# team-ergo-unipi/ergo_uvo

Hardware: AMD Instinct MI355X
Metric: stereo frame-pairs/sec (detect+match+pose) @1920x1080, 3k kpts (higher is better)
Workload: dtype f32+f64

## Files before the change

### ergo_uvo_amd/csrc/surf.hip

```cpp
#include "uvo_ctx.h"
#include <type_traits>
#include <string.h>
#include "uvo_math.h"
#include <algorithm>
#include <utility>
#include <vector>
#include <string>

namespace uvo {

struct ImgPair { const uint8_t* img[2]; int32_t* sum[2]; int32_t* planes[2]; int pw, pstride; int* cand_n; int* big_n; int* surv_n; };
struct AreaTab;
struct CandOut { uvo_keypoint* cand[2]; int* count; int cap; };
struct SurvOut { Survivor* list; int* count; int cap; };
static_assert(sizeof(Survivor) == 128, "a survivor record is 32 words");
struct SortArgs { const uvo_keypoint* cand[2]; const int* cand_n; uvo_keypoint* out[2]; int* out_n[2]; int* rank; int cap;
                  int4* big_par; int* big_n; int* gate_nqa; int gate_min_features; };
struct DescArgs { const uint8_t* img[2]; uvo_keypoint* kps[2]; float* desc[2]; const int* n[2]; const float* DW;
                  const int4* big_par; const int* big_n; const int* big_large; int cap;
                  const AreaTab* tabs; const int* iscale;
                  int extended;
                  const int32_t* sum[2]; const float* ori_w; int* ori_drop; };
struct LaneArgs { ImgPair ip; int32_t* part; SurvOut sv; CandOut out; SortArgs sa; DescArgs da; uint8_t* patch; const int4* big_in; int4* big_out; int* big_large; };
struct LanePair { LaneArgs a[2]; };
// ... 454 lines not shown

template <int O, int L>
__device__ __forceinline__ float plane_pp(ImgRsrc rs, int voff, int pw, int pstride)
{
    using LC = LayerC<OctC<O>::size(L)>;
#define SVP(dy, dx) (int)__builtin_amdgcn_raw_buffer_load_b32(rs, voff + 4 * ((dx) >> 2) + plane_written<(dy), (dx)>(), 4 * ((((dy) & 3) * 4 + ((dx) & 3)) * pstride + ((dy) >> 2) * pw), 0)
    UVO_HESSIAN_CONSTS(LC);
    float pp;
    UVO_HESSIAN_PP(SVP, pp)
    return pp;
}
template <int O, int L>
__device__ __forceinline__ float plane_det(ImgRsrc rs, int voff, int pw, int pstride, float pp)
{
    using LC = LayerC<OctC<O>::size(L)>;
    UVO_HESSIAN_CONSTS(LC);
    float det;
    UVO_HESSIAN_DXY(SVP, pp, det)
#undef SVP
    return det;
}
template <int O, int TW, int TH, int NT, class OP>
__device__ __forceinline__ void det_layers_p3(const int32_t* __restrict__ planes, int pw, int pstride, float* __restrict__ sdet,
                                              const OP& op, int px0, int py0, float skip_thr)
{
    using OC = OctC<O>;
    constexpr int Q = OC::STEP / 4;
    const ImgRsrc rs = img_rsrc(reinterpret_cast<const uint8_t*>(planes), 16 * pstride * 4);
    const int tid = lane_tid();
#pragma unroll
    for (int it = 0; it < (TW * TH + NT - 1) / NT; it++) {
        const int sidx = tid + it * NT;
        if ((it + 1) * NT > TW * TH && sidx >= TW * TH) break;
        const int ry = sidx / TW, rx = sidx - ry * TW;
        bool ok[3]; int voff[3]; float pp[3], det[3];
#pragma unroll
        for (int l = 0; l < 3; l++) {
            const int m = l == 0 ? OC::margin(1) : l == 1 ? OC::margin(2) : OC::margin(3);
            const auto& lp = op.L[l + 1];
            const int oi = py0 + ry - m, oj = px0 + rx - m;
            ok[l] = oi >= 0 && oi < lp.samples_i && oj >= 0 && oj < lp.samples_j;
            voff[l] = ok[l] ? 4 * ((oi * Q) * pw + oj * Q) : 0x7FFFFFF0;
        }
        pp[0] = plane_pp<O, 1>(rs, voff[0], pw, pstride);
        pp[1] = plane_pp<O, 2>(rs, voff[1], pw, pstride);
        pp[2] = plane_pp<O, 3>(rs, voff[2], pw, pstride);
        const bool n0 = ok[0] && pp[0] > skip_thr, n1 = ok[1] && pp[1] > skip_thr, n2 = ok[2] && pp[2] > skip_thr;
        det[0] = ok[0] ? kDetBelow : 0.f; det[1] = ok[1] ? kDetBelow : 0.f; det[2] = ok[2] ? kDetBelow : 0.f;
        if (n0 || n1 || n2) {
            const float d0 = plane_det<O, 1>(rs, n0 ? voff[0] : 0x7FFFFFF0, pw, pstride, pp[0]);
            const float d1 = plane_det<O, 2>(rs, n1 ? voff[1] : 0x7FFFFFF0, pw, pstride, pp[1]);
            const float d2 = plane_det<O, 3>(rs, n2 ? voff[2] : 0x7FFFFFF0, pw, pstride, pp[2]);
            if (n0) det[0] = d0;
            if (n1) det[1] = d1;
            if (n2) det[2] = d2;
        }
#pragma unroll
        for (int l = 0; l < 3; l++) sdet[(l * TH + ry) * TW + rx] = det[l];
    }
}


template <int TW, int TH>
struct NmsLds { static constexpr int kList = 3 * ((TW - 1) / 2) * ((TH - 1) / 2), kWords = kList + 2; };

#ifndef UVO_STAMPS
#define UVO_STAMPS 0
#endif
__device__ long long* g_hess_stamps = nullptr;
__device__ __forceinline__ void hess_stamp(int k, long long v = -1)
{
#if UVO_STAMPS
    long long* st = g_hess_stamps;
    if (st && threadIdx.x == 0) st[((size_t)blockIdx.y * gridDim.x + blockIdx.x) * 8 + k] = v >= 0 ? v : (long long)wall_clock64();
#endif
}
template <int TW, int TH>
__device__ __forceinline__ void nms_zero(unsigned* s_list) { if (lane_tid() == 0) reinterpret_cast<int*>(s_list + NmsLds<TW, TH>::kList)[0] = 0; }
template <int TW, int TH, int NT, class OP>
__device__ __forceinline__ void nms_survivors(const float* __restrict__ sdet, unsigned* __restrict__ s_list, const OP& op, float thr,
                                              int px0, int py0, int im, const SurvOut& sv)
{
    const int tid = lane_tid();
    int* s_n = reinterpret_cast<int*>(s_list + NmsLds<TW, TH>::kList);
    static_assert((TW & (TW - 1)) == 0 && NT % TW == 0 && TW <= 64, "tile width: a power of two that divides the workgroup, a row within a wave");
    constexpr int G = NT / TW, ITER = (TH - 2 + G - 1) / G;
    const int rx = tid & (TW - 1), g = tid / TW;
    const int j = px0 + rx;
    float col[3][ITER + 2];
#pragma unroll
    for (int l = 0; l < 3; l++)
#pragma unroll
        for (int k = 0; k < ITER + 2; k++) col[l][k] = sdet[(l * TH + min(g * ITER + k, TH - 1)) * TW + rx];
    float cmax = col[0][1];
#pragma unroll
    for (int l = 0; l < 3; l++)
#pragma unroll
        for (int k = 0; k < ITER; k++) cmax = fmaxf(cmax, col[l][k + 1]);
    if (__any(cmax > thr)) {
    float m3[3][ITER], m3l[3][ITER], m3r[3][ITER];
#pragma unroll
    for (int l = 0; l < 3; l++)
#pragma unroll
        for (int k = 0; k < ITER; k++) {
            const float v = fmaxf(fmaxf(col[l][k], col[l][k + 1]), col[l][k + 2]);
            m3[l][k] = v;
            m3l[l][k] = __int_as_float(__builtin_amdgcn_update_dpp(__float_as_int(v), __float_as_int(v), 0x138, 0xF, 0xF, false));
            m3r[l][k] = __int_as_float(__builtin_amdgcn_update_dpp(__float_as_int(v), __float_as_int(v), 0x130, 0xF, 0xF, false));
        }
#pragma unroll
    for (int l = 0; l < 3; l++) {
        const int L = l + 1;
        const int m = op.nms_margin[l];
        const bool col_ok = op.L[L].samples_i != 0 && op.L[L + 1].samples_i != 0 && rx >= 1 && rx <= TW - 2 && j >= m && j < op.cols - m;
#pragma unroll
        for (int k = 0; k < ITER; k++) {
            const int ry = g * ITER + k + 1, i = py0 + ry;
            const float val0 = col[l][k + 1];
            float nb = fmaxf(fmaxf(col[l][k], col[l][k + 2]), fmaxf(m3l[l][k], m3r[l][k]));
            if (L <= 2) nb = fmaxf(nb, fmaxf(m3[l + 1][k], fmaxf(m3l[l + 1][k], m3r[l + 1][k])));
            if (L >= 2) nb = fmaxf(nb, fmaxf(m3[l - 1][k], fmaxf(m3l[l - 1][k], m3r[l - 1][k])));
            const bool is_max = col_ok && ry <= TH - 2 && i >= m && i < op.rows - m && val0 > thr && val0 > nb;
            if (is_max) s_list[atomicAdd(&s_n[0], 1)] = (unsigned)L | ((unsigned)ry << 8) | ((unsigned)rx << 16);
        }
    }
    }
    hess_stamp(5);
    __syncthreads();
    hess_stamp(6);
    const int nloc = s_n[0];
    if (nloc == 0) return;
    if (tid == 0) s_n[1] = atomicAdd(sv.count, nloc);
    __syncthreads();
    hess_stamp(7);
    const int base = s_n[1];
    for (int e = tid; e < nloc * 32; e += NT) {
        const int t = e >> 5, wd = e & 31;
        if (base + t >= sv.cap) continue;
        Survivor* r = sv.list + base + t;
        const unsigned ent = s_list[t];
        const int L = ent & 255u, ry = (ent >> 8) & 255u, rx = ent >> 16;
        int val;
        if (wd < 5) val = wd == 0 ? im : wd == 1 ? op.octave : wd == 2 ? L : wd == 3 ? py0 + ry : px0 + rx;
        else {
            const int q = wd - 5, row = q / 9, nb9 = q - row * 9;
            const float* d = sdet + ((L - 2 + row) * TH + ry + nb9 / 3 - 1) * TW + rx + nb9 % 3 - 1;
            const bool have = (row == 0 && L >= 2) || row == 1 || (row == 2 && L <= 2);
            val = have ? __float_as_int(*d) : 0;
        }
        reinterpret_cast<int*>(r)[wd] = val;
    }
}

static const int kFinishPerWg = 16;
__global__ __launch_bounds__(256) void k_hessian_finish(LanePair lp, const OctavePat* __restrict__ ops, int w, int h)
{
    const LaneArgs& LA = lp.a[blockIdx.y]; const SurvOut& sv = LA.sv; const ImgPair& ip = LA.ip; const CandOut& out = LA.out;
    __shared__ uvo_keypoint s_kp[2][kFinishPerWg];
    __shared__ int s_cnt[2], s_base[2];
    const int grp = threadIdx.x >> 4, k = threadIdx.x & 15;
    const int n = min(*sv.count, sv.cap);
    if (blockIdx.x == 0 && threadIdx.x == 0 && *sv.count > sv.cap) atomicAdd(&out.count[0], out.cap + 1);
    if (blockIdx.x * kFinishPerWg >= n) return;
    if (threadIdx.x < 2) s_cnt[threadIdx.x] = 0;
    __syncthreads();
    const int sw = w + 1;
#pragma unroll 1
    for (int rd = 0; rd < kFinishPerWg / 16; rd++) {
        const int t = blockIdx.x * kFinishPerWg + rd * 16 + grp;
        if (t >= n) continue;
        const Survivor* r = sv.list + t;
        const int im = r->im, L = r->L, i = r->i, j = r->j;
        const OctavePat& op = ops[r->octave];
        const int step = op.step;
        const int32_t* __restrict__ gsum = ip.sum[im];
        auto exact_det = [&](const LayerPat& lo, int ii, int jj) {
            const int oi = ii - lo.margin, oj = jj - lo.margin;
            float d = 0.f;
            if (oi >= 0 && oi < lo.samples_i && oj >= 0 && oj < lo.samples_j) {
                const int32_t* o = gsum + (size_t)(oi * step) * sw + oj * step;
                float dx, dy, dxy;
                haar_response(lo, [&](int yy, int xx) { return o[(size_t)yy * sw + xx]; }, &dx, &dy, &dxy);
                d = dx * dy - 0.81f * dxy * dxy;
            }
            return d;
        };
        float v2[2];
#pragma unroll
        for (int q = 0; q < 2; q++) {
            const int e = k + 16 * q;
            v2[q] = r->n9[e < 27 ? e : 0];
        }
#pragma unroll 1
        for (int q = 0; q < 2; q++) {
            const int e = k + 16 * q;
            if (e >= 27) continue;
            const int row = e / 9, nb = e - row * 9;
            const bool outer = (L == 1 && row == 0) || (L == 3 && row == 2);
            if (outer || v2[q] == kDetBelow) v2[q] = exact_det(op.L[L - 1 + row], i + nb / 3 - 1, j + nb % 3 - 1);
        }
        const int g0 = (threadIdx.x & 63) & ~15;
        float N9[3][9];
#pragma unroll
        for (int e = 0; e < 27; e++) N9[e / 9][e % 9] = __shfl(v2[e / 16], g0 + (e & 15));
        if (k != 0) continue;
        const float val0 = N9[1][4];
        if (L != 2) {
            bool is_max = true;
#pragma unroll
            for (int b = 0; b < 9; b++) is_max = is_max && (val0 > (L == 1 ? N9[0][b] : N9[2][b]));
            if (!is_max) continue;
        }
        const LayerPat& lp = op.L[L];
        float dx, dy;
        {
            const int32_t* o = gsum + (size_t)((i - lp.margin) * step) * sw + (j - lp.margin) * step;
            haar_response(lp, [&](int yy, int xx) { return o[(size_t)yy * sw + xx]; }, &dx, &dy, nullptr);
        }
        const int ds = lp.size - op.L[L - 1].size;
        uvo_keypoint kp;
        bool ok;
        switch (step) {
        case 1:  ok = make_keypoint<1>(N9, val0, dx + dy, i, j, lp.size, ds, op.octave, w, h, &kp); break;
        case 2:  ok = make_keypoint<2>(N9, val0, dx + dy, i, j, lp.size, ds, op.octave, w, h, &kp); break;
        case 4:  ok = make_keypoint<4>(N9, val0, dx + dy, i, j, lp.size, ds, op.octave, w, h, &kp); break;
        default: ok = make_keypoint<8>(N9, val0, dx + dy, i, j, lp.size, ds, op.octave, w, h, &kp); break;
        }
        if (ok) s_kp[im][atomicAdd(&s_cnt[im], 1)] = kp;
    }
    __syncthreads();
    if (threadIdx.x < 2 && s_cnt[threadIdx.x] > 0) s_base[threadIdx.x] = atomicAdd(&out.count[threadIdx.x], s_cnt[threadIdx.x]);
    __syncthreads();
    for (int e = threadIdx.x; e < 2 * kFinishPerWg; e += 256) {
        const int im = e / kFinishPerWg, q = e - im * kFinishPerWg;
        if (q < s_cnt[im] && s_base[im] + q < out.cap) out.cand[im][s_base[im] + q] = s_kp[im][q];
    }
}

#define UVO_FILL(quads, nt) (((quads) + (nt) - 1) / (nt) <= 6 ? ((quads) + (nt) - 1) / (nt) : 4)
template <int O, int TW, int TH, int NT, class OP>
__device__ __forceinline__ void hessian_nms_c_tile(const ImgPair& ip, int w, int h, const OP& op, float thr, const SurvOut& sv,
                                                   int bx, int by, int im, unsigned char* smem)
{
    using OC = OctC<O>;
    constexpr int STEP = OC::STEP;
    constexpr int TWs = OctTile<O, TW>::TWs;
    constexpr int THs = (TH - 1) * STEP + (OC::HI - OC::LO) + 1;
    constexpr int PW = OctTile<O, TW>::PW;
    const int tid = lane_tid();
    const int sw = w + 1;
    const int32_t* __restrict__ gsum = ip.sum[im];
    float* sdet = reinterpret_cast<float*>(smem);
    int32_t* stile = reinterpret_cast<int32_t*>(smem + sizeof(float) * 3 * TH * TW);

    const int px0 = bx * (TW - 2) - 1, py0 = by * (TH - 2) - 1;
    const int sx0 = px0 * STEP + OC::LO, sy0 = py0 * STEP + OC::LO;
    constexpr int QPR = OctTile<O, TW>::TWq / 4, kQuads = THs * QPR, kFill = UVO_FILL(kQuads, NT), kQ = NT / QPR, kR = NT % QPR;
    static_assert(STEP == 1 || STEP == 2, "tile fill handles octaves 0 and 1");
    static_assert(OctTile<O, TW>::TWq < kSumPad && STEP - OC::LO < kSumPad, "integral slack too small for the tile overshoot");
    int fidx = tid, fty = tid / QPR, fq = tid - fty * QPR;
#pragma unroll 1
    for (int i0 = 0; i0 < kQuads; i0 += NT * kFill) {
        SumQuad v[kFill];
        int dst[kFill];
#pragma unroll
        for (int u = 0; u < kFill; u++) {
            const bool in = fidx < kQuads;
            const int gy = min(max(sy0 + fty, 0), h), gx = sx0 + 4 * fq;
            v[u] = *reinterpret_cast<const SumQuad*>(gsum + (in ? gy * sw + gx : 0));
            dst[u] = in ? fty * STEP * PW + (4 / STEP) * fq : -1;
            fidx += NT; fq += kR; fty += kQ;
            if (fq >= QPR) { fq -= QPR; fty++; }
        }
#pragma unroll
        for (int u = 0; u < kFill; u++) {
            if (dst[u] < 0) continue;
            if constexpr (STEP == 1) {
                *reinterpret_cast<int4*>(stile + dst[u]) = make_int4(v[u].a, v[u].b, v[u].c, v[u].d);
            } else {
                *reinterpret_cast<int2*>(stile + dst[u]) = make_int2(v[u].a, v[u].c);
                *reinterpret_cast<int2*>(stile + dst[u] + PW) = make_int2(v[u].b, v[u].d);
            }
        }
    }
    nms_zero<TW, TH>(reinterpret_cast<unsigned*>(stile + THs * STEP * PW));
    __syncthreads();
    hess_stamp(1);
    det_layer_c<O, 1, TW, TH, NT>(stile, sdet, op, px0, py0, thr);
    det_layer_c<O, 2, TW, TH, NT>(stile, sdet, op, px0, py0, thr);
    det_layer_c<O, 3, TW, TH, NT>(stile, sdet, op, px0, py0, thr);
    __syncthreads();
    hess_stamp(2);
    nms_survivors<TW, TH, NT>(sdet, reinterpret_cast<unsigned*>(stile + THs * STEP * PW), op, thr, px0, py0, im, sv);
}
template <int O, int TW, int TH, int NT>
__global__ __launch_bounds__(NT) void k_hessian_nms_c(LanePair lp, int w, int h, OctavePat op, float thr)
{
    extern __shared__ __align__(16) unsigned char smem[];
    const LaneArgs& LA = UVO_LANE_OF(lp, blockIdx.z);
    hessian_nms_c_tile<O, TW, TH, NT>(LA.ip, w, h, op, thr, LA.sv, blockIdx.x, blockIdx.y, UVO_LANE_IM(blockIdx.z), smem);
}

template <int O, int TW, int TH, int NT>
__global__ __launch_bounds__(NT) void k_hessian_nms_p(LanePair lp, int w, int h, OctavePat op, float thr)
{
    __shared__ float sdet[3 * TH * TW];
    __shared__ unsigned s_list[NmsLds<TW, TH>::kWords];
    const LaneArgs& LA = UVO_LANE_OF(lp, blockIdx.z); const ImgPair& ip = LA.ip; const SurvOut& sv = LA.sv;
    const int im = UVO_LANE_IM(blockIdx.z);
    const int px0 = blockIdx.x * (TW - 2) - 1, py0 = blockIdx.y * (TH - 2) - 1;
    det_layer_p<O, 1, TW, TH, NT>(ip.planes[im], ip.pw, ip.pstride, sdet, op, px0, py0, thr);
    det_layer_p<O, 2, TW, TH, NT>(ip.planes[im], ip.pw, ip.pstride, sdet, op, px0, py0, thr);
    det_layer_p<O, 3, TW, TH, NT>(ip.planes[im], ip.pw, ip.pstride, sdet, op, px0, py0, thr);
    nms_zero<TW, TH>(s_list);
    __syncthreads();
    nms_survivors<TW, TH, NT>(sdet, s_list, op, thr, px0, py0, im, sv);
}

static const int kP23Threads = 512;
struct P23Grid { int nbx2, nb2, nbx3, nb3; };
template <class OP>
__device__ __forceinline__ void hessian_nms_p23_tile(const ImgPair& ip, const OP& op2, const OP& op3, float thr, const SurvOut& sv,
                                                     bool oct3, int bx, int by, int im, float* sdet, unsigned* s_list)
{
    constexpr int TW2 = 32, TH2 = 16, TW3 = 16, TH3 = 16;
    static_assert(TW3 * TH3 <= TW2 * TH2 && NmsLds<TW3, TH3>::kWords <= NmsLds<TW2, TH2>::kWords, "octave 3 reuses octave 2's LDS");
    if (!oct3) {
        const int px0 = bx * (TW2 - 2) - 1, py0 = by * (TH2 - 2) - 1;
        det_layers_p3<2, TW2, TH2, kP23Threads>(ip.planes[im], ip.pw, ip.pstride, sdet, op2, px0, py0, thr);
        nms_zero<TW2, TH2>(s_list);
        __syncthreads();
        hess_stamp(2);
        nms_survivors<TW2, TH2, kP23Threads>(sdet, s_list, op2, thr, px0, py0, im, sv);
    } else {
        const int px0 = bx * (TW3 - 2) - 1, py0 = by * (TH3 - 2) - 1;
        det_layers_p3<3, TW3, TH3, kP23Threads>(ip.planes[im], ip.pw, ip.pstride, sdet, op3, px0, py0, thr);
        nms_zero<TW3, TH3>(s_list);
        __syncthreads();
        hess_stamp(2);
        nms_survivors<TW3, TH3, kP23Threads>(sdet, s_list, op3, thr, px0, py0, im, sv);
    }
}
static const int kP23SdetFloats = 3 * 16 * 32;
static const int kO1TileRows = 18;
struct HessGrid { int nbx0, nb0, nbx1, nb1; P23Grid g; };
template <int TW, int TH>
__global__ __launch_bounds__(kP23Threads) void k_hessian_nms_all(LanePair lp, int w, int h, HessDims hd, float thr,
                                                                 const uint32_t* __restrict__ order)
{
    extern __shared__ __align__(16) unsigned char smem[];
    const LaneArgs& LA = UVO_LANE_OF(lp, blockIdx.y); const ImgPair& ip = LA.ip;
    SurvOut sv = LA.sv;
    asm volatile("" : "+s"(sv.list), "+s"(sv.count), "+s"(sv.cap));
    const int im = UVO_LANE_IM(blockIdx.y);
    const unsigned e = order[blockIdx.x];
    const int kind = e >> 30, bx = e & 0x3FFF, by = (e >> 14) & 0x3FFF;
    hess_stamp(0); hess_stamp(4, kind);
    if (kind == 0) hessian_nms_c_tile<0, TW, TH, kP23Threads>(ip, w, h, hd.o[0], thr, sv, bx, by, im, smem);
    else if (kind == 1) hessian_nms_c_tile<1, 32, kO1TileRows, kP23Threads>(ip, w, h, hd.o[1], thr, sv, bx, by, im, smem);
    else {
        float* sdet = reinterpret_cast<float*>(smem);
        hessian_nms_p23_tile(ip, hd.o[2], hd.o[3], thr, sv, kind == 3, bx, by, im, sdet, reinterpret_cast<unsigned*>(sdet + kP23SdetFloats));
    }
    hess_stamp(3);
}

__global__ __launch_bounds__(256) void k_probe_hold(int ticks)
{
    extern __shared__ int probe_lds[];
    if (threadIdx.x == 0) probe_lds[0] = ticks;
    const long long t0 = wall_clock64();
    while (wall_clock64() - t0 < ticks) __builtin_amdgcn_s_sleep(16);
}

__global__ void k_hessian_layer_debug(const int32_t* gsum, int w, int h, LayerPat lp, int step, int rows, int cols,
                                      float* det, float* trace)
{
    int j = blockIdx.x * blockDim.x + threadIdx.x, i = blockIdx.y;
    if (j >= lp.samples_j || i >= lp.samples_i) return;
    const int sw = w + 1;
    const int32_t* o = gsum + (size_t)(i * step) * sw + j * step;
    float dx, dy, dxy;
    haar_response(lp, [&](int yy, int xx) { return o[(size_t)yy * sw + xx]; }, &dx, &dy, &dxy);
    size_t pos = (size_t)(i + lp.margin) * cols + (j + lp.margin);
    det[pos] = dx * dy - 0.81f * dxy * dxy;
    trace[pos] = dx + dy;
}

// ... 1011 lines not shown
    static bool attr_dev[64] = {false};
    bool& attr_set = attr_dev[c->device & 63];
    if (!attr_set) {
        hipError_t e = hipFuncSetAttribute(reinterpret_cast<const void*>(kern), hipFuncAttributeMaxDynamicSharedMemorySize, (int)lds);
        if (e != hipSuccess) return e;
        attr_set = true;
    }
    hipLaunchKernelGGL(kern, grid, dim3(NT), lds, c->stream, lp, w, h, op, thr);
    return hipGetLastError();
}

struct MergedGrid { int nbx0, nb0, nbx1, nb1, nb23, total; P23Grid g; };
static const int kMergedTW0 = 64, kMergedTH0 = 32, kMergedTW1 = 32;
static MergedGrid merged_grid(const OctavePat* ops)
{
    constexpr int TW0 = kMergedTW0, TH0 = kMergedTH0, TW1 = kMergedTW1, TH1 = kO1TileRows;
    MergedGrid m;
    m.nbx0 = (ops[0].cols + TW0 - 3) / (TW0 - 2); m.nb0 = m.nbx0 * ((ops[0].rows + TH0 - 3) / (TH0 - 2));
    m.nbx1 = (ops[1].cols + TW1 - 3) / (TW1 - 2); m.nb1 = m.nbx1 * ((ops[1].rows + TH1 - 3) / (TH1 - 2));
    m.g.nbx2 = (ops[2].cols + 32 - 3) / (32 - 2); m.g.nb2 = m.g.nbx2 * ((ops[2].rows + 16 - 3) / (16 - 2));
    m.g.nbx3 = (ops[3].cols + 16 - 3) / (16 - 2); m.g.nb3 = m.g.nbx3 * ((ops[3].rows + 16 - 3) / (16 - 2));
    m.nb23 = m.g.nb2 + m.g.nb3; m.total = m.nb0 + m.nb1 + m.nb23;
    return m;
}
static bool merged_launch(const Ctx* c)
{
    static const bool split_env = getenv("UVO_HESSIAN_SPLIT") != nullptr;
    return c->p.SURF_OCTAVES_NUMBER == 4 && !split_env;
}

uvo_status surf_prepare(Ctx* c, int w, int h)
{
    if (c->p.SURF_OCTAVES_NUMBER < 1 || c->p.SURF_OCTAVES_NUMBER > 4 || c->p.SURF_OCTAVES_LAYERS != 3) {
        c->err = "SURF: supported nOctaves 1..4, nOctaveLayers 3";
        return UVO_INVALID_ARG;
    }
    OctavePat ops[4];
    memset(ops, 0, sizeof(ops));
    for (int o = 0; o < c->p.SURF_OCTAVES_NUMBER; o++) make_octave(o, c->p.SURF_OCTAVES_LAYERS, w, h, &ops[o]);
    if (!c->d_octpat) UVO_HIP_TRY(c, hipMalloc(&c->d_octpat, sizeof(ops)));
    if (c->h_octpat.size() != sizeof(ops) || memcmp(c->h_octpat.data(), ops, sizeof(ops)) != 0) {
        UVO_HIP_TRY(c, hipStreamSynchronize(c->stream));
        c->h_octpat.assign(reinterpret_cast<const unsigned char*>(ops), reinterpret_cast<const unsigned char*>(ops) + sizeof(ops));
        UVO_HIP_TRY(c, hipMemcpyAsync(c->d_octpat, c->h_octpat.data(), sizeof(ops), hipMemcpyHostToDevice, c->stream));
        UVO_HIP_TRY(c, hipStreamSynchronize(c->stream));
    }
    if (!merged_launch(c)) return UVO_OK;
    const MergedGrid m = merged_grid(ops);
    const int nb0 = m.nb0, nb1 = m.nb1, nb23 = m.nb23, total = m.total;
    if (nb0 > 0x3FFF || nb1 > 0x3FFF || nb23 > 0x3FFF) { c->err = "SURF: image too large for the merged detection launch's tile table"; return UVO_INVALID_ARG; }
    const int ng[3] = { nb0, nb1, nb23 }, ngroups = total;
    if ((int)c->h_hess_order.size() != ngroups || c->hess_order_key[0] != nb0 || c->hess_order_key[1] != nb1 || c->hess_order_key[2] != nb23) {
        std::vector<std::pair<double, uint32_t>> pos;
        pos.reserve((size_t)ngroups);
        for (int k = 0; k < 3; k++) for (int i = 0; i < ng[k]; i++) {
            uint32_t e;
            if (k == 0) e = (0u << 30) | ((uint32_t)(i / m.nbx0) << 14) | (uint32_t)(i % m.nbx0);
            else if (k == 1) e = (1u << 30) | ((uint32_t)(i / m.nbx1) << 14) | (uint32_t)(i % m.nbx1);
            else if (i < m.g.nb2) e = (2u << 30) | ((uint32_t)(i / m.g.nbx2) << 14) | (uint32_t)(i % m.g.nbx2);
            else e = (3u << 30) | ((uint32_t)((i - m.g.nb2) / m.g.nbx3) << 14) | (uint32_t)((i - m.g.nb2) % m.g.nbx3);
            pos.emplace_back((i + 0.5) / ng[k] + k * 1e-9, e);
        }
        std::sort(pos.begin(), pos.end());
        c->h_hess_order.resize((size_t)ngroups);
        for (int b = 0; b < ngroups; b++) c->h_hess_order[(size_t)b] = pos[(size_t)b].second;
        UVO_HIP_TRY(c, hipStreamSynchronize(c->stream));
        if (c->d_hess_order_cap < (size_t)ngroups) {
            if (c->d_hess_order) (void)hipFree(c->d_hess_order);
            c->d_hess_order = nullptr; c->d_hess_order_cap = 0;
            UVO_HIP_TRY(c, hipMalloc(reinterpret_cast<void**>(&c->d_hess_order), sizeof(uint32_t) * (size_t)ngroups));
            c->d_hess_order_cap = (size_t)ngroups;
        }
        UVO_HIP_TRY(c, hipMemcpyAsync(c->d_hess_order, c->h_hess_order.data(), sizeof(uint32_t) * (size_t)ngroups, hipMemcpyHostToDevice, c->stream));
        UVO_HIP_TRY(c, hipStreamSynchronize(c->stream));
        c->hess_order_key[0] = nb0; c->hess_order_key[1] = nb1; c->hess_order_key[2] = nb23;
    }
    return UVO_OK;
}

uvo_status surf_detect_lanes(Ctx* c, Ctx* c2, int nimg, int gate_min_features)
{
    const int w = c->img_w, h = c->img_h;
    if (c2 && (nimg != 2 || c2->img_w != w || c2->img_h != h || !c->p.SURF_UPRIGHT)) { c->err = "two-pair launch: upright SURF on two image pairs of one size"; return UVO_INVALID_ARG; }
    UVO_TRY(surf_prepare(c, w, h));
    if (c2) { const uvo_status st2 = surf_prepare(c2, w, h); if (st2 != UVO_OK) { c->err = c2->err; return st2; } }
    const LanePair lp = lane_pair(c, c2, nimg, gate_min_features);
    const int nim = c2 ? 2 * nimg : nimg, nlanes = c2 ? 2 : 1;
    UVO_TRY(surf_integral_lanes(c, lp, nim));
    const float thr = (float)c->p.SURF_MIN_HESSIAN;
    {
        OctavePat ops[4];
        memset(ops, 0, sizeof(ops));
        for (int o = 0; o < c->p.SURF_OCTAVES_NUMBER; o++) make_octave(o, c->p.SURF_OCTAVES_LAYERS, w, h, &ops[o]);
        const bool merged = merged_launch(c);
        if (merged) {
            constexpr int TW0 = kMergedTW0, TH0 = kMergedTH0, TW1 = kMergedTW1, TH1 = kO1TileRows;
            constexpr int THs0 = (TH0 - 1) * OctC<0>::STEP + (OctC<0>::HI - OctC<0>::LO) + 1, THs1 = (TH1 - 1) * OctC<1>::STEP + (OctC<1>::HI - OctC<1>::LO) + 1;
            constexpr size_t lds0 = sizeof(float) * 3 * TW0 * TH0 + sizeof(int32_t) * (size_t)THs0 * OctC<0>::STEP * OctTile<0, TW0>::PW + sizeof(unsigned) * NmsLds<TW0, TH0>::kWords;
            constexpr size_t lds1 = sizeof(float) * 3 * TW1 * TH1 + sizeof(int32_t) * (size_t)THs1 * OctC<1>::STEP * OctTile<1, TW1>::PW + sizeof(unsigned) * NmsLds<TW1, TH1>::kWords;
            constexpr size_t lds = lds0 > lds1 ? lds0 : lds1;
            static_assert(lds <= 54600, "three blocks of the merged detection launch must fit a CU's 160 KB of LDS");
            const MergedGrid mg = merged_grid(ops);
            const HessGrid hg = { mg.nbx0, mg.nb0, mg.nbx1, mg.nb1, mg.g };
            const int total = mg.total;
            auto kern = k_hessian_nms_all<TW0, TH0>;
            static bool attr_dev[64] = {false};
            bool& attr_set = attr_dev[c->device & 63];
            if (!attr_set) { UVO_HIP_TRY(c, hipFuncSetAttribute(reinterpret_cast<const void*>(kern), hipFuncAttributeMaxDynamicSharedMemorySize, (int)lds)); attr_set = true; }
            StageTimer t(c, ST_HESSIAN_O0);
            static const size_t lds_pad = getenv("UVO_HESS_LDS") ? (size_t)atoi(getenv("UVO_HESS_LDS")) : 0;
            const size_t lds_launch = lds_pad > lds ? lds_pad : lds;
            if (lds_pad > lds) { static bool once = false; if (!once) { (void)hipFuncSetAttribute(reinterpret_cast<const void*>(kern), hipFuncAttributeMaxDynamicSharedMemorySize, (int)lds_launch); once = true; } }
            static const char* stamps_path = UVO_STAMPS ? getenv("UVO_HESS_STAMPS") : nullptr;
            static long long* d_stamps = nullptr; static size_t stamps_n = 0;
            if (stamps_path && c->lane_id == 0 && !c->master) {
                if (!d_stamps) { stamps_n = (size_t)total * 4 * 8; (void)hipMalloc(reinterpret_cast<void**>(&d_stamps), sizeof(long long) * stamps_n); (void)hipMemcpyToSymbol(HIP_SYMBOL(g_hess_stamps), &d_stamps, sizeof(d_stamps)); }
                (void)hipMemsetAsync(d_stamps, 0, sizeof(long long) * stamps_n, c->stream);
            }
            HessDims hd;
            for (int o = 0; o < 4; o++) {
                OctDims& d = hd.o[o];
                for (int l = 0; l < 5; l++) { d.L[l].samples_i = ops[o].L[l].samples_i; d.L[l].samples_j = ops[o].L[l].samples_j; }
                d.rows = ops[o].rows; d.cols = ops[o].cols; d.octave = ops[o].octave;
                for (int l = 0; l < 3; l++) d.nms_margin[l] = ops[o].nms_margin[l];
            }
            Ctx::TraceRec* trh = (c->trace_on && c->trace_cur >= 0) ? &c->trace[c->trace_cur] : nullptr;
            if (trh) (void)hipEventRecord(trh->ev[6], c->stream);
            hipLaunchKernelGGL(kern, dim3(total, nim), dim3(kP23Threads), lds_launch, c->stream, lp, w, h, hd, thr, c->d_hess_order);
            if (trh) { (void)hipEventRecord(trh->ev[7], c->stream); trh->det_marked = true; }
            if (stamps_path && d_stamps && c->lane_id == 0 && !c->master) {
                std::vector<long long> hs(stamps_n);
                (void)hipStreamSynchronize(c->stream);
                (void)hipMemcpy(hs.data(), d_stamps, sizeof(long long) * stamps_n, hipMemcpyDeviceToHost);
                if (FILE* f = fopen(stamps_path, "w")) {
                    fprintf(f, "block,im,kind,t_start,t_filled,t_det,t_end,t_scan,t_scanbar,t_atomic\n");
                    for (int y = 0; y < nim; y++) for (int b = 0; b < total; b++) { const long long* r = hs.data() + ((size_t)y * total + b) * 8; fprintf(f, "%d,%d,%lld,%lld,%lld,%lld,%lld,%lld,%lld,%lld\n", b, y, r[4], r[0], r[1], r[2], r[3], r[5], r[6], r[7]); }
                    fclose(f);
                }
            }
            UVO_HIP_TRY(c, hipGetLastError());
        }
        for (int o = 0; o < c->p.SURF_OCTAVES_NUMBER && !merged; o++) {
            StageTimer t(c, ST_HESSIAN_O0 + o);
            const OctavePat& op = ops[o];
            hipError_t e;
            if (o == 0)      e = launch_hessian_c<0, 64, 24, 512>(c, lp, nim, op, thr);
            else if (o == 1) e = launch_hessian_c<1, 32, 24, 512>(c, lp, nim, op, thr);
            else if (o == 2) e = launch_hessian_p<2, 32, 16, 512>(c, lp, nim, op, thr);
            else             e = launch_hessian_p<3, 16, 16, 256>(c, lp, nim, op, thr);
            UVO_HIP_TRY(c, e);
        }
        {
            StageTimer t(c, ST_HESSIAN_O0 + c->p.SURF_OCTAVES_NUMBER - 1);
            hipLaunchKernelGGL(k_hessian_finish, dim3((c->surv_cap + kFinishPerWg - 1) / kFinishPerWg, nlanes), dim3(256), 0, c->stream, lp, static_cast<const OctavePat*>(c->d_octpat), w, h);
            UVO_HIP_TRY(c, hipGetLastError());
        }
        static const int probe_thin = getenv("UVO_PROBE_THIN_US") ? atoi(getenv("UVO_PROBE_THIN_US")) : 0, probe_fat = getenv("UVO_PROBE_FAT_US") ? atoi(getenv("UVO_PROBE_FAT_US")) : 0;
        if (probe_thin > 0) hipLaunchKernelGGL(k_probe_hold, dim3(1), dim3(64), 64, c->stream, probe_thin * 100);
        if (probe_fat > 0) {
            static bool once = false;
            if (!once) { (void)hipFuncSetAttribute(reinterpret_cast<const void*>(k_probe_hold), hipFuncAttributeMaxDynamicSharedMemorySize, 53000); once = true; }
            hipLaunchKernelGGL(k_probe_hold, dim3(768), dim3(256), 53000, c->stream, probe_fat * 100);
        }
    }
    {
        StageTimer t(c, ST_SORT);
        hipLaunchKernelGGL(k_order, dim3(1, nim), dim3(kOrderThreads), 0, c->stream, lp, c->d_area_iscale);
        if (c->cap > kOrderCap) {
            const int tiles_max = ((c->cap + 255) / 256) * ((c->cap + kSortChunk - 1) / kSortChunk);
            hipLaunchKernelGGL(k_rank_partial, dim3(tiles_max < 512 ? tiles_max : 512, nim), dim3(256), 0, c->stream, lp);
            hipLaunchKernelGGL(k_rank_scatter, dim3((c->cap + 255) / 256, nim), dim3(256), 0, c->stream, lp);
            hipLaunchKernelGGL(k_big_sort, dim3(nim), dim3(1024), 0, c->stream, lp, c->cap, c->d_area_iscale);
        }
        UVO_HIP_TRY(c, hipGetLastError());
    }
    {
        StageTimer t(c, ST_DESCRIPTOR);
        const size_t lds_small = sizeof(float) * 21 * ((kSmallWin + 3) | 1), lds_big = sizeof(float) * 4 * kBigRow;
        if (c->p.SURF_UPRIGHT) {
            const int nbig = 1024;
            static const int desc_part = getenv("UVO_DESC_PART") ? atoi(getenv("UVO_DESC_PART")) : 0;
            static const char* dstamps_path = UVO_STAMPS ? getenv("UVO_DESC_STAMPS") : nullptr;
            static long long* d_dstamps = nullptr; const size_t dstamps_n = (size_t)4 * 16384 * 8;
            const bool dstamp = dstamps_path && c->lane_id == 0 && !c->master && nim == 2;
            if (dstamp) {
                if (!d_dstamps) { (void)hipMalloc(reinterpret_cast<void**>(&d_dstamps), sizeof(long long) * dstamps_n); (void)hipMemcpyToSymbol(HIP_SYMBOL(g_desc_stamps), &d_dstamps, sizeof(d_dstamps)); }
                (void)hipMemsetAsync(d_dstamps, 0, sizeof(long long) * dstamps_n, c->stream);
            }
            const Ctx* hm = c->master ? c->master : c;
            static const int fixed_grid = getenv("UVO_DESC_GRID") ? atoi(getenv("UVO_DESC_GRID")) : 0;
            int nsmall = hm->kp_hint > 0 ? ((hm->kp_hint + hm->kp_hint / 4 + 255) & ~255) : c->cap;
            if (fixed_grid != 0) nsmall = fixed_grid < 0 ? c->cap : fixed_grid;
            nsmall = nsmall < 512 ? 512 : (nsmall > c->cap ? c->cap : nsmall);
            static const int desc_order = getenv("UVO_DESC_ORDER") ? atoi(getenv("UVO_DESC_ORDER")) : 2;
            static const int nbig_env = getenv("UVO_DESC_NBIG") ? atoi(getenv("UVO_DESC_NBIG")) : 0;
            const int nbig_l = nbig_env > 0 ? nbig_env : nbig;
            hipLaunchKernelGGL(k_descriptor64, dim3((nbig_l + nsmall) * nim), dim3(256), lds_small > lds_big ? lds_small : lds_big, c->stream, lp, w, h, nbig_l, desc_part, nim, desc_order);
            if (dstamp && d_dstamps) {
                std::vector<long long> hs(dstamps_n);
                (void)hipStreamSynchronize(c->stream);
                (void)hipMemcpy(hs.data(), d_dstamps, sizeof(long long) * dstamps_n, hipMemcpyDeviceToHost);
                if (FILE* f = fopen(dstamps_path, "w")) {
                    fprintf(f, "im,k,t_start,t_kp,t_ready,t_horiz,t_vert,t_end,win,kind\n");
                    for (int y = 0; y < 2; y++) for (int k = 0; k < 16384; k++) { const long long* r = hs.data() + ((size_t)y * 16384 + k) * 8; if (r[0]) fprintf(f, "%d,%d,%lld,%lld,%lld,%lld,%lld,%lld,%lld,%lld\n", y, k, r[0], r[1], r[2], r[3], r[4], r[5], r[6], r[7]); }
                    fclose(f);
                }
                if (FILE* f = fopen((std::string(dstamps_path) + ".big").c_str(), "w")) {
                    fprintf(f, "im,task,t_start,t_horiz,t_end,win,kind\n");
                    for (int y = 0; y < 2; y++) for (int k = 0; k < 16384; k++) { const long long* r = hs.data() + ((size_t)(2 + y) * 16384 + k) * 8; if (r[0] && r[2]) fprintf(f, "%d,%d,%lld,%lld,%lld,%lld,%lld\n", y, k, r[0], r[1], r[2], r[6], r[7]); }
                    fclose(f);
                }
            }
            hipLaunchKernelGGL(k_descriptor64_big_finish, dim3(1024, nim), dim3(256), 0, c->stream, lp);
        } else {
            const DescArgs& da = lp.a[0].da;
            const size_t lds_rot = sizeof(float) * 21 * (kMaxWin + 1);
            static bool rot_attr_dev[64] = {false};
            bool& rot_attr = rot_attr_dev[c->device & 63];
            if (!rot_attr) { UVO_HIP_TRY(c, hipFuncSetAttribute(reinterpret_cast<const void*>(k_descriptor_rot), hipFuncAttributeMaxDynamicSharedMemorySize, (int)lds_rot)); rot_attr = true; }
            hipLaunchKernelGGL(k_surf_orientation, dim3((c->cap + 3) / 4, nimg), dim3(256), 0, c->stream, da, w, h);
            hipLaunchKernelGGL(k_descriptor_rot, dim3(2048, nimg), dim3(256), lds_rot, c->stream, da, w, h);
        }
        UVO_HIP_TRY(c, hipGetLastError());
    }
    return UVO_OK;
}
uvo_status surf_detect(Ctx* c, int nimg, int gate_min_features) { return surf_detect_lanes(c, nullptr, nimg, gate_min_features); }

uvo_status surf_hessian_layer_debug(Ctx* c, int octave, int layer, float* det, float* trace)
{
    const int w = c->img_w, h = c->img_h;
    if (octave < 0 || octave > 3 || layer < 0 || layer > 4 || w <= 0) { c->err = "hessian_layer: bad octave/layer or no image"; return UVO_INVALID_ARG; }
    OctavePat op;
    make_octave(octave, 3, w, h, &op);
    size_t n = (size_t)op.rows * op.cols;
    float *d_det = nullptr, *d_tr = nullptr;
    UVO_HIP_TRY(c, hipMalloc(&d_det, sizeof(float) * n * 2));
    d_tr = d_det + n;
    UVO_HIP_TRY(c, hipMemsetAsync(d_det, 0, sizeof(float) * n * 2, c->stream));
    const LayerPat& lp = op.L[layer];
    if (lp.samples_i > 0) {
        dim3 g((lp.samples_j + 255) / 256, lp.samples_i);
        hipLaunchKernelGGL(k_hessian_layer_debug, g, dim3(256), 0, c->stream, c->d_sum[0], w, h, lp, op.step, op.rows, op.cols, d_det, d_tr);
    }
    UVO_HIP_TRY(c, hipMemcpyAsync(det, d_det, sizeof(float) * n, hipMemcpyDeviceToHost, c->stream));
    UVO_HIP_TRY(c, hipMemcpyAsync(trace, d_tr, sizeof(float) * n, hipMemcpyDeviceToHost, c->stream));
    UVO_HIP_TRY(c, hipStreamSynchronize(c->stream));
    (void)hipFree(d_det);
    return UVO_OK;
}

}
```

Before: 3135.

## Restructure Hessian finish kernel with early outer-layer rejection and lane-balanced Haar evaluation

```diff
diff --git a/ergo_uvo_amd/csrc/surf.hip b/ergo_uvo_amd/csrc/surf.hip
--- a/ergo_uvo_amd/csrc/surf.hip
+++ b/ergo_uvo_amd/csrc/surf.hip
@@ -630,8 +630,61 @@
     }
 }
 
-static const int kFinishPerWg = 16;
-__global__ __launch_bounds__(256) void k_hessian_finish(LanePair lp, const OctavePat* __restrict__ ops, int w, int h)
+
+__device__ __forceinline__ void haar_half_dxdy(const LayerPat& lp, const int32_t* __restrict__ o, int sw, float* pdx, float* pdy)
+{
+    const int32_t* r1 = o + (size_t)lp.dy1[0] * sw; const int32_t* r2 = o + (size_t)lp.dy2[0] * sw;
+    const int x0 = lp.dx1[0], x1 = lp.dx2[0], x2 = lp.dx2[1], x3 = lp.dx2[2];
+    const int a0 = r1[x0], a1 = r1[x1], a2 = r1[x2], a3 = r1[x3], b0 = r2[x0], b1 = r2[x1], b2 = r2[x2], b3 = r2[x3];
+    const int32_t* c1 = o + lp.dx1[3]; const int32_t* c2 = o + lp.dx2[3];
+    const size_t y0 = (size_t)lp.dy1[3] * sw, y1 = (size_t)lp.dy2[3] * sw, y2 = (size_t)lp.dy2[4] * sw, y3 = (size_t)lp.dy2[5] * sw;
+    const int e0 = c1[y0], e1 = c1[y1], e2 = c1[y2], e3 = c1[y3], f0 = c2[y0], f1 = c2[y1], f2 = c2[y2], f3 = c2[y3];
+    double d = 0;
+    d += (float)(a0 + b1 - b0 - a1) * lp.w[0];
+    d += (float)(a1 + b2 - b1 - a2) * lp.w[1];
+    d += (float)(a2 + b3 - b2 - a3) * lp.w[2];
+    *pdx = (float)d;
+    d = 0;
+    d += (float)(e0 + f1 - e1 - f0) * lp.w[3];
+    d += (float)(e1 + f2 - e2 - f1) * lp.w[4];
+    d += (float)(e2 + f3 - e3 - f2) * lp.w[5];
+    *pdy = (float)d;
+}
+__device__ __forceinline__ float haar_half_dxy(const LayerPat& lp, const int32_t* __restrict__ o, int sw)
+{
+    double d = 0;
+#pragma unroll
+    for (int k = 6; k < 10; k++) {
+        const int32_t* r1 = o + (size_t)lp.dy1[k] * sw; const int32_t* r2 = o + (size_t)lp.dy2[k] * sw;
+        const int v = r1[lp.dx1[k]] + r2[lp.dx2[k]] - r2[lp.dx1[k]] - r1[lp.dx2[k]];
+        d += (float)v * lp.w[k];
+    }
+    return (float)d;
+}
+
+enum { FC_L1, FC_L2, FC_L3, FC_REJECTED, FC_MAXIMA, FC_KEYPOINTS, FC_OUTER_IN, FC_OUTER_OUT, FC_OUTER_SKIP, FC_OUTER_SKIP_CORNER, FC_OUTER_DXY_A,
+       FC_OUTER_DXY_B, FC_BELOW_EVAL, FC_BELOW_READ_REJECTED, FC_BELOW_UNREAD, FC_LOADS, FC_UNITS, FC_PASSES, FC_N };
+__device__ unsigned long long* g_finish_cnt = nullptr;
+__device__ __forceinline__ void finish_count(int k, unsigned v = 1)
+{
+#if UVO_STAMPS
+    unsigned long long* fc = g_finish_cnt;
+    if (fc) atomicAdd(fc + k, (unsigned long long)v);
+#endif
+}
+
+#ifndef UVO_FINISH_PAT_LDS
+#define UVO_FINISH_PAT_LDS 1
+#endif
+#ifndef UVO_FINISH_PER_WG
+#define UVO_FINISH_PER_WG 16
+#endif
+#ifndef UVO_FINISH_GRID
+#define UVO_FINISH_GRID 768
+#endif
+static const int kFinishPerWg = UVO_FINISH_PER_WG, kFinishThreads = 16 * kFinishPerWg, kFinishGrid = UVO_FINISH_GRID;
+static_assert(kFinishThreads % 64 == 0 && kFinishThreads <= 256, "whole waves of four survivor groups");
+__global__ __launch_bounds__(kFinishThreads) void k_hessian_finish(LanePair lp, const OctavePat* __restrict__ ops, int w, int h)
 {
     const LaneArgs& LA = lp.a[blockIdx.y]; const SurvOut& sv = LA.sv; const ImgPair& ip = LA.ip; const CandOut& out = LA.out;
     __shared__ uvo_keypoint s_kp[2][kFinishPerWg];
@@ -640,78 +693,165 @@
     const int n = min(*sv.count, sv.cap);
     if (blockIdx.x == 0 && threadIdx.x == 0 && *sv.count > sv.cap) atomicAdd(&out.count[0], out.cap + 1);
     if (blockIdx.x * kFinishPerWg >= n) return;
-    if (threadIdx.x < 2) s_cnt[threadIdx.x] = 0;
-    __syncthreads();
+#if UVO_FINISH_PAT_LDS
+    __shared__ int s_pat[sizeof(OctavePat) * 4 / sizeof(int)];
+    const OctavePat* pats = reinterpret_cast<const OctavePat*>(s_pat);
+#else
+    const OctavePat* pats = ops;
+#endif
     const int sw = w + 1;
 #pragma unroll 1
-    for (int rd = 0; rd < kFinishPerWg / 16; rd++) {
-        const int t = blockIdx.x * kFinishPerWg + rd * 16 + grp;
-        if (t >= n) continue;
-        const Survivor* r = sv.list + t;
-        const int im = r->im, L = r->L, i = r->i, j = r->j;
-        const OctavePat& op = ops[r->octave];
+    for (int t0 = blockIdx.x * kFinishPerWg; t0 < n; t0 += gridDim.x * kFinishPerWg) {
+    if (threadIdx.x < 2) s_cnt[threadIdx.x] = 0;
+    const int t = t0 + grp;
+    const Survivor* r = sv.list + min(t, n - 1);
+    const int im = r->im, L = r->L, i = r->i, j = r->j, oct = r->octave;
+    float val[2];
+#pragma unroll
+    for (int q = 0; q < 2; q++) val[q] = r->n9[k + 16 * q < 27 ? k + 16 * q : 0];
+#if UVO_FINISH_PAT_LDS
+    if (t0 == (int)blockIdx.x * kFinishPerWg)
+        for (int e = threadIdx.x; e < (int)(sizeof(OctavePat) * 4 / sizeof(int)); e += kFinishThreads) s_pat[e] = reinterpret_cast<const int*>(ops)[e];
+#endif
+    __syncthreads();
+    if (t < n) {
+        const OctavePat& op = pats[oct];
         const int step = op.step;
         const int32_t* __restrict__ gsum = ip.sum[im];
-        auto exact_det = [&](const LayerPat& lo, int ii, int jj) {
-            const int oi = ii - lo.margin, oj = jj - lo.margin;
-            float d = 0.f;
-            if (oi >= 0 && oi < lo.samples_i && oj >= 0 && oj < lo.samples_j) {
-                const int32_t* o = gsum + (size_t)(oi * step) * sw + oj * step;
-                float dx, dy, dxy;
-                haar_response(lo, [&](int yy, int xx) { return o[(size_t)yy * sw + xx]; }, &dx, &dy, &dxy);
-                d = dx * dy - 0.81f * dxy * dxy;
-            }
-            return d;
+        const int g0 = (threadIdx.x & 63) & ~15;
+        const int outer_row = L == 1 ? 0 : L == 3 ? 2 : -1;
+        auto locate = [&](int e, const LayerPat*& lo, const int32_t*& o) {
+            const int row = e / 9, nb = e - row * 9;
+            lo = &op.L[L - 1 + row];
+            const int oi = i + nb / 3 - 1 - lo->margin, oj = j + nb % 3 - 1 - lo->margin;
+            const bool in = oi >= 0 && oi < lo->samples_i && oj >= 0 && oj < lo->samples_j;
+            o = gsum + (in ? (size_t)(oi * step) * sw + oj * step : 0);
+            return in;
         };
-        float v2[2];
+        float hdx[2] = { 0.f, 0.f }, hdy[2] = { 0.f, 0.f }, hdxy[2] = { 0.f, 0.f };
+        bool have_dxdy[2] = { false, false }, have_dxy[2] = { false, false }, need_dxdy[2] = { false, false }, need_dxy[2] = { false, false };
+        const float val0 = __shfl(val[0], g0 + 13);
+        if (k == 0) finish_count(FC_L1 + L - 1);
+
+        bool alive = true;
+        if (L != 2) {
+            const int qo = L == 1 ? 0 : 1, eo = k + 16 * qo;
+            const bool mine = eo < 27 && eo / 9 == outer_row;
+            bool fail = false, a_dxdy = false, a_dxy = false;
+            float dx = 0.f, dy = 0.f, dxy = 0.f;
+            if (mine) {
+                const LayerPat* lo; const int32_t* o;
+                if (locate(eo, lo, o)) {
+                    haar_half_dxdy(*lo, o, sw, &dx, &dy);
+                    a_dxdy = true;
+                    const float p = dx * dy;
+                    finish_count(FC_OUTER_IN); finish_count(FC_LOADS, 16);
+                    if (!(val0 > p)) {
+                        dxy = haar_half_dxy(*lo, o, sw);
+                        a_dxy = true;
+                        fail = !(val0 > p - 0.81f * dxy * dxy);
+                        finish_count(FC_OUTER_DXY_A); finish_count(FC_LOADS, 16);
+                    } else {
+                        finish_count(FC_OUTER_SKIP);
+                        const int nb = eo % 9;
+                        if (nb == 0 || nb == 2 || nb == 6 || nb == 8) finish_count(FC_OUTER_SKIP_CORNER);
+                    }
+                } else {
+                    fail = !(val0 > 0.f);
+                    finish_count(FC_OUTER_OUT);
+                }
+            }
+            alive = ((__ballot(fail) >> g0) & 0xFFFFull) == 0;
+            if (mine) {
+                if (L == 1) { hdx[0] = dx; hdy[0] = dy; hdxy[0] = dxy; have_dxdy[0] = a_dxdy; have_dxy[0] = a_dxy; if (!a_dxdy) val[0] = 0.f; }
+                else        { hdx[1] = dx; hdy[1] = dy; hdxy[1] = dxy; have_dxdy[1] = a_dxdy; have_dxy[1] = a_dxy; if (!a_dxdy) val[1] = 0.f; }
+            }
+            if (k == 0) finish_count(alive ? FC_MAXIMA : FC_REJECTED);
+        } else if (k == 0) finish_count(FC_MAXIMA);
+#if UVO_STAMPS
 #pragma unroll
         for (int q = 0; q < 2; q++) {
-            const int e = k + 16 * q;
-            v2[q] = r->n9[e < 27 ? e : 0];
-        }
-#pragma unroll 1
-        for (int q = 0; q < 2; q++) {
-            const int e = k + 16 * q;
-            if (e >= 27) continue;
-            const int row = e / 9, nb = e - row * 9;
-            const bool outer = (L == 1 && row == 0) || (L == 3 && row == 2);
-            if (outer || v2[q] == kDetBelow) v2[q] = exact_det(op.L[L - 1 + row], i + nb / 3 - 1, j + nb % 3 - 1);
-        }
-        const int g0 = (threadIdx.x & 63) & ~15;
-        float N9[3][9];
-#pragma unroll
-        for (int e = 0; e < 27; e++) N9[e / 9][e % 9] = __shfl(v2[e / 16], g0 + (e & 15));
-        if (k != 0) continue;
-        const float val0 = N9[1][4];
-        if (L != 2) {
-            bool is_max = true;
-#pragma unroll
-            for (int b = 0; b < 9; b++) is_max = is_max && (val0 > (L == 1 ? N9[0][b] : N9[2][b]));
-            if (!is_max) continue;
-        }
-        const LayerPat& lp = op.L[L];
-        float dx, dy;
-        {
-            const int32_t* o = gsum + (size_t)((i - lp.margin) * step) * sw + (j - lp.margin) * step;
-            haar_response(lp, [&](int yy, int xx) { return o[(size_t)yy * sw + xx]; }, &dx, &dy, nullptr);
-        }
-        const int ds = lp.size - op.L[L - 1].size;
-        uvo_keypoint kp;
-        bool ok;
-        switch (step) {
-        case 1:  ok = make_keypoint<1>(N9, val0, dx + dy, i, j, lp.size, ds, op.octave, w, h, &kp); break;
-        case 2:  ok = make_keypoint<2>(N9, val0, dx + dy, i, j, lp.size, ds, op.octave, w, h, &kp); break;
-        case 4:  ok = make_keypoint<4>(N9, val0, dx + dy, i, j, lp.size, ds, op.octave, w, h, &kp); break;
-        default: ok = make_keypoint<8>(N9, val0, dx + dy, i, j, lp.size, ds, op.octave, w, h, &kp); break;
-        }
-        if (ok) s_kp[im][atomicAdd(&s_cnt[im], 1)] = kp;
+            const int e = k + 16 * q, row = e / 9, nb = e - row * 9;
+            if (e < 27 && row != outer_row && val[q] == kDetBelow) {
+                const bool readp = row == 1 || nb == 1 || nb == 3 || nb == 4 || nb == 5 || nb == 7;
+                if (!readp) finish_count(FC_BELOW_UNREAD); else if (!alive) finish_count(FC_BELOW_READ_REJECTED);
+            }
+        }
+#endif
+        if (alive) {
+#pragma unroll
+            for (int q = 0; q < 2; q++) {
+                const int e = k + 16 * q, row = e / 9, nb = e - row * 9;
+                if (e >= 27) continue;
+                const bool readp = row == 1 || nb == 1 || nb == 3 || nb == 4 || nb == 5 || nb == 7;
+                if (row == outer_row) need_dxy[q] = readp && have_dxdy[q] && !have_dxy[q];
+                else if (e == 13) need_dxdy[q] = true;
+                else if (readp && val[q] == kDetBelow) {
+                    const LayerPat* lo; const int32_t* o;
+                    if (locate(e, lo, o)) { need_dxdy[q] = need_dxy[q] = true; finish_count(FC_BELOW_EVAL); } else val[q] = 0.f;
+                }
+                if (row == outer_row && need_dxy[q]) finish_count(FC_OUTER_DXY_B);
+            }
+            unsigned long long units = 0;
+#pragma unroll
+            for (int q = 0; q < 2; q++) {
+                units |= ((__ballot(need_dxdy[q]) >> g0) & 0xFFFFull) << (32 * q);
+                units |= ((__ballot(need_dxy[q]) >> g0) & 0xFFFFull) << (32 * q + 16);
+            }
+            unsigned long long rest = units;
+            for (int pass = 0; rest != 0; pass++) {
+                unsigned long long m = rest;
+                for (int s = 0; s < k; s++) m &= m - 1;
+                float ra = 0.f, rb = 0.f;
+                if (m != 0) {
+                    const int u = __ffsll((long long)m) - 1, e = (u & 15) + 16 * (u >> 5);
+                    const LayerPat* lo; const int32_t* o;
+                    locate(e, lo, o);
+                    if (e == 13) o = gsum + (size_t)((i - lo->margin) * step) * sw + (j - lo->margin) * step;
+                    if (u & 16) ra = haar_half_dxy(*lo, o, sw); else haar_half_dxdy(*lo, o, sw, &ra, &rb);
+                    finish_count(FC_UNITS); finish_count(FC_LOADS, 16);
+                }
+                if (k == 0) finish_count(FC_PASSES);
+#pragma unroll
+                for (int q = 0; q < 2; q++) {
+                    const int u0 = 32 * q + k, u1 = u0 + 16;
+                    const int n0 = __popcll(units & ((1ull << u0) - 1)), n1 = __popcll(units & ((1ull << u1) - 1));
+                    const float ta = __shfl(ra, g0 + (n0 & 15)), tb = __shfl(rb, g0 + (n0 & 15)), tc = __shfl(ra, g0 + (n1 & 15));
+                    if (need_dxdy[q] && (n0 >> 4) == pass) { hdx[q] = ta; hdy[q] = tb; have_dxdy[q] = true; }
+                    if (need_dxy[q] && (n1 >> 4) == pass) { hdxy[q] = tc; have_dxy[q] = true; }
+                }
+                for (int s = 0; s < 16 && rest != 0; s++) rest &= rest - 1;
+            }
+#pragma unroll
+            for (int q = 0; q < 2; q++)
+                if (have_dxdy[q] && have_dxy[q]) val[q] = hdx[q] * hdy[q] - 0.81f * hdxy[q] * hdxy[q];
+            const float trace = __shfl(hdx[0] + hdy[0], g0 + 13);
+            float N9[3][9];
+#pragma unroll
+            for (int e = 0; e < 27; e++) N9[e / 9][e % 9] = __shfl(val[e / 16], g0 + (e & 15));
+            if (k == 0) {
+                const LayerPat& cl = op.L[L];
+                const int ds = cl.size - op.L[L - 1].size;
+                uvo_keypoint kp;
+                bool ok;
+                switch (step) {
+                case 1:  ok = make_keypoint<1>(N9, val0, trace, i, j, cl.size, ds, op.octave, w, h, &kp); break;
+                case 2:  ok = make_keypoint<2>(N9, val0, trace, i, j, cl.size, ds, op.octave, w, h, &kp); break;
+                case 4:  ok = make_keypoint<4>(N9, val0, trace, i, j, cl.size, ds, op.octave, w, h, &kp); break;
+                default: ok = make_keypoint<8>(N9, val0, trace, i, j, cl.size, ds, op.octave, w, h, &kp); break;
+                }
+                if (ok) { s_kp[im][atomicAdd(&s_cnt[im], 1)] = kp; finish_count(FC_KEYPOINTS); }
+            }
+        }
     }
     __syncthreads();
     if (threadIdx.x < 2 && s_cnt[threadIdx.x] > 0) s_base[threadIdx.x] = atomicAdd(&out.count[threadIdx.x], s_cnt[threadIdx.x]);
     __syncthreads();
-    for (int e = threadIdx.x; e < 2 * kFinishPerWg; e += 256) {
+    for (int e = threadIdx.x; e < 2 * kFinishPerWg; e += kFinishThreads) {
         const int im = e / kFinishPerWg, q = e - im * kFinishPerWg;
         if (q < s_cnt[im] && s_base[im] + q < out.cap) out.cand[im][s_base[im] + q] = s_kp[im][q];
+    }
+    __syncthreads();
     }
 }
 
@@ -2029,7 +2169,28 @@
         }
         {
             StageTimer t(c, ST_HESSIAN_O0 + c->p.SURF_OCTAVES_NUMBER - 1);
-            hipLaunchKernelGGL(k_hessian_finish, dim3((c->surv_cap + kFinishPerWg - 1) / kFinishPerWg, nlanes), dim3(256), 0, c->stream, lp, static_cast<const OctavePat*>(c->d_octpat), w, h);
+            static const char* counts_path = UVO_STAMPS ? getenv("UVO_FINISH_COUNTS") : nullptr;
+            static unsigned long long* d_fcnt = nullptr;
+            const bool counting = counts_path && c->lane_id == 0 && !c->master;
+            if (counting) {
+                if (!d_fcnt) { (void)hipMalloc(reinterpret_cast<void**>(&d_fcnt), sizeof(unsigned long long) * FC_N); (void)hipMemcpyToSymbol(HIP_SYMBOL(g_finish_cnt), &d_fcnt, sizeof(d_fcnt)); }
+                (void)hipMemsetAsync(d_fcnt, 0, sizeof(unsigned long long) * FC_N, c->stream);
+            }
+            hipLaunchKernelGGL(k_hessian_finish, dim3(std::min((c->surv_cap + kFinishPerWg - 1) / kFinishPerWg, kFinishGrid), nlanes), dim3(kFinishThreads), 0, c->stream, lp, static_cast<const OctavePat*>(c->d_octpat), w, h);
+            if (counting && d_fcnt) {
+                static const char* const names[FC_N] = { "survivors_L1", "survivors_L2", "survivors_L3", "rejected", "maxima", "keypoints", "outer_in_range", "outer_out_of_range",
+                    "outer_decided_by_dxdy", "outer_decided_by_dxdy_corner", "outer_dxy_phase_a", "outer_dxy_phase_b", "below_evaluated", "below_read_of_rejected", "below_unread",
+                    "integral_loads", "units_phase_b", "passes_phase_b" };
+                unsigned long long hc[FC_N];
+                (void)hipStreamSynchronize(c->stream);
+                (void)hipMemcpy(hc, d_fcnt, sizeof(hc), hipMemcpyDeviceToHost);
+                if (FILE* f = fopen(counts_path, "w")) {
+                    fprintf(f, "{");
+                    for (int q = 0; q < FC_N; q++) fprintf(f, "%s\"%s\": %llu", q ? ", " : "", names[q], hc[q]);
+                    fprintf(f, "}\n");
+                    fclose(f);
+                }
+            }
             UVO_HIP_TRY(c, hipGetLastError());
         }
         static const int probe_thin = getenv("UVO_PROBE_THIN_US") ? atoi(getenv("UVO_PROBE_THIN_US")) : 0, probe_fat = getenv("UVO_PROBE_FAT_US") ? atoi(getenv("UVO_PROBE_FAT_US")) : 0;
```

Result: no change. 3138 (median of 2 runs) (+0.1%).
